# wu-kan/multicore-hw2

Hardware: AMD Instinct MI355X
Metric: queries/sec (exact 1-NN, bit-exact vs v0), m=1024 n=16777216 k=16 (higher is better)
Workload: dtype f32 results (f16 MFMA filter + f32 exact re-rank)

## Files before the change

### include/knn_mi355x.h

```cpp
#ifndef KNN_MI355X_H
#define KNN_MI355X_H

#ifdef __cplusplus
extern "C" {
#endif

void cudaCallback(int k, int m, int n, float *searchPoints, float *referencePoints,
                  int **results);

long long knn_trim(void);

typedef struct knn_index knn_index;

enum {
    KNN_OK = 0,
    KNN_EINVAL = -1,
    KNN_ENODEV = -2,
    KNN_EHIP = -3,
    KNN_ENOMEM = -4
};

#define KNN_KEY_INIT 0x7F80000000000000ull

int knn_device_count(void);
const char *knn_last_error(void);
const char *knn_version(void);

int knn_index_create(knn_index **out, int device, int k, long long n_local, const float *refs,
                     int refs_on_device, long long base_index, void *stream);
void knn_index_destroy(knn_index *idx);

typedef struct knn_geom knn_geom;
int knn_geom_create(knn_geom **out, int k, long long n_global, int nranks, const float *sample_host, long long samples,
                    int seed_tiles);
void knn_geom_destroy(knn_geom *g);
int knn_geom_info(const knn_geom *g, long long out[8]);
long long knn_geom_first_cell(const knn_geom *g, int rank);
int knn_geom_assign(const knn_geom *g, int device, const float *rows_dev, long long n, int *owner_dev, void *stream);
int knn_index_create_sharded(knn_index **out, int device, const knn_geom *g, int rank, long long n_local, const float *refs_dev,
                             const unsigned *gids_dev, void *stream);
int knn_index_seed_export(knn_index *idx, void *layer_dev, void *stream);
int knn_index_seed_attach(knn_index *idx, const void *layer_dev);

int knn_keys_init(int device, unsigned long long *keys_dev, int m, void *stream);

int knn_index_query_keys(knn_index *idx, int m, const float *queries_dev,
                         unsigned long long *keys_dev, void *stream);

int knn_index_query_keys_slot(knn_index *idx, int slot, int m, const float *queries_dev,
                              unsigned long long *keys_dev, void *stream);

#define KNN_QUERY_INIT_KEYS 1u
int knn_index_query_keys_ex(knn_index *idx, int slot, int m, const float *queries_dev,
                            unsigned long long *keys_dev, void *stream, unsigned flags);

int knn_index_query(knn_index *idx, int slot, int m, const float *queries_dev, unsigned long long *keys_dev,
                    int *indices_dev, void *stream, unsigned flags);

int knn_keys_allreduce_min(int ndev, const int *devices, unsigned long long *const *keys_dev, int m,
                           void *const *streams);

int knn_keys_to_indices(int device, const unsigned long long *keys_dev, int m, int *out_dev,
                        void *stream);

int knn_index_query_host(knn_index *idx, int m, const float *queries_host, int *out_host);

int knn_index_query_topk(knn_index *idx, int slot, int m, int K, const float *queries_dev, unsigned long long *keys_dev,
                         int *indices_dev, void *stream, unsigned flags);
int knn_keys_topk_merge(int device, int m, int K, const unsigned long long *a_dev, unsigned long long *b_dev, void *stream);
int knn_index_query_topk_host(knn_index *idx, int m, int K, const float *queries_host, int *indices_host, float *dist2_host);

int knn_set_option(const char *name, long long value);
long long knn_get_option(const char *name);

int knn_index_last_stats(knn_index *idx, long long stats[4]);

int knn_index_debug_counters(knn_index *idx, long long out[4]);

int knn_debug_shard_policy(int k, int m, long long n, int ndev);
int knn_debug_plan_shard(int k, int m, long long rows, long long out[4]);
int knn_debug_u8_row(int k, const float *row, const float *centre, float scale, double amax, unsigned char *codes, double out[2]);
int knn_debug_u8_bin_row(int k, const float *row, const float *centre, float scale, const float *w, unsigned char *codes, double *err);
int knn_debug_u8_bin_threshold(int k, const unsigned short *b_bits, float dup, float ratio, float er, float nmax, float w1, float *thr);

int knn_debug_scan_plan(int num_cu, int blocks_per_cu, unsigned nitems, int m, long long out[8]);
int knn_debug_scan_plan_ex(int num_cu, int blocks_per_cu, unsigned nitems, int m, int self_lists, long long out[8]);
int knn_debug_cells_query_plan(const long long in[14], long long out[28]);
int knn_debug_cells_topk_plan(const long long in[20], long long out[25]);
int knn_debug_seed_kth(const float *seed, int nseed, const float *wide, int nwide, int K, int pw, float *out);
int knn_debug_topk_gate(int k, float sigma, double amax, double bmax, double nmax, double u, double mq, double out[3]);
int knn_debug_filter_query_plan(const long long in[11], long long out[49]);

int knn_debug_filter_scores(knn_index *idx, int m, const float *queries_dev, float *scores_dev,
                            float *qnorm_dev, double consts[8]);

int knn_index_timing(knn_index *idx, int enable);
int knn_index_timing_read(knn_index *idx, int *launches, double *total_ms);

int knn_synth_fill_device(int device, float *dst_dev, long long count, unsigned long long seed,
                          long long first, void *stream);

#ifdef __cplusplus
}
#endif
#endif
```

### multicore_hw2_amd/__init__.py

```python
import ctypes
import os
import sys

import numpy as np

__all__ = ["lib", "lib_path", "cudaCallback", "KnnIndex", "KnnGeom", "KnnError", "KEY_INIT", "set_option",
           "get_option", "trim", "device_count", "EXPORTED_SYMBOLS", "shard_bounds", "keys_topk_merge"]

KEY_INIT = 0x7F80000000000000

EXPORTED_SYMBOLS = [
    "cudaCallback", "knn_device_count", "knn_last_error", "knn_version", "knn_index_create",
    "knn_index_destroy", "knn_keys_init", "knn_index_query_keys", "knn_keys_to_indices",
    "knn_index_query_host", "knn_set_option", "knn_get_option", "knn_index_last_stats",
    "knn_synth_fill_device", "knn_index_timing", "knn_index_timing_read",
    "knn_debug_filter_scores", "knn_index_query_keys_slot", "knn_trim", "knn_keys_allreduce_min",
    "knn_index_query_keys_ex", "knn_index_debug_counters", "knn_debug_scan_plan", "knn_debug_scan_plan_ex", "knn_debug_cells_query_plan", "knn_debug_cells_topk_plan", "knn_debug_seed_kth", "knn_debug_topk_gate", "knn_debug_filter_query_plan", "knn_debug_shard_policy", "knn_debug_plan_shard", "knn_debug_u8_row", "knn_debug_u8_bin_row", "knn_debug_u8_bin_threshold", "knn_index_query",
    "knn_geom_create", "knn_geom_destroy", "knn_geom_info", "knn_geom_assign", "knn_index_create_sharded",
    "knn_index_seed_export", "knn_index_seed_attach", "knn_geom_first_cell",
    "knn_index_query_topk", "knn_keys_topk_merge", "knn_index_query_topk_host",
]
QUERY_INIT_KEYS = 1

_HERE = os.path.dirname(os.path.abspath(__file__))
lib_path = os.environ.get("KNN_MI355X_LIB") or os.path.join(_HERE, "libknn_mi355x.so")
_lib = None


class KnnError(RuntimeError):
    pass


def lib():
    global _lib
    if _lib is not None:
        return _lib
    if not os.path.exists(lib_path):
        raise KnnError(f"{lib_path} is missing: run `python -c 'import __graft_entry__ as g; g.build()'` "
                       "(there is no CPU fallback)")
    if "torch" not in sys.modules and os.environ.get("KNN_MI355X_NO_TORCH") != "1":
        try:
            import torch
        except ImportError:
            pass
    L = ctypes.CDLL(lib_path)
    c_int, c_ll, c_vp, c_ull = ctypes.c_int, ctypes.c_longlong, ctypes.c_void_p, ctypes.c_ulonglong
    L.cudaCallback.argtypes = [c_int, c_int, c_int, c_vp, c_vp, ctypes.POINTER(ctypes.POINTER(c_int))]
    L.cudaCallback.restype = None
    L.knn_device_count.restype = c_int
    L.knn_last_error.restype = ctypes.c_char_p
    L.knn_version.restype = ctypes.c_char_p
    L.knn_index_create.argtypes = [ctypes.POINTER(c_vp), c_int, c_int, c_ll, c_vp, c_int, c_ll, c_vp]
    L.knn_index_destroy.argtypes = [c_vp]
    L.knn_index_destroy.restype = None
    L.knn_keys_init.argtypes = [c_int, c_vp, c_int, c_vp]
    L.knn_index_query_keys.argtypes = [c_vp, c_int, c_vp, c_vp, c_vp]
    L.knn_index_query_keys_slot.argtypes = [c_vp, c_int, c_int, c_vp, c_vp, c_vp]
    L.knn_index_query_keys_ex.argtypes = [c_vp, c_int, c_int, c_vp, c_vp, c_vp, ctypes.c_uint]
    L.knn_index_query.argtypes = [c_vp, c_int, c_int, c_vp, c_vp, c_vp, c_vp, ctypes.c_uint]
    L.knn_keys_to_indices.argtypes = [c_int, c_vp, c_int, c_vp, c_vp]
    L.knn_index_query_host.argtypes = [c_vp, c_int, c_vp, c_vp]
    L.knn_set_option.argtypes = [ctypes.c_char_p, c_ll]
    L.knn_get_option.argtypes = [ctypes.c_char_p]
    L.knn_get_option.restype = c_ll
    L.knn_index_last_stats.argtypes = [c_vp, ctypes.POINTER(c_ll)]
    L.knn_synth_fill_device.argtypes = [c_int, c_vp, c_ll, c_ull, c_ll, c_vp]
    L.knn_index_timing.argtypes = [c_vp, c_int]
    L.knn_debug_filter_scores.argtypes = [c_vp, c_int, c_vp, c_vp, c_vp, ctypes.POINTER(ctypes.c_double)]
    L.knn_index_timing_read.argtypes = [c_vp, ctypes.POINTER(c_int), ctypes.POINTER(ctypes.c_double)]
    L.knn_geom_create.argtypes = [ctypes.POINTER(c_vp), c_int, c_ll, c_int, c_vp, c_ll, c_int]
    L.knn_geom_destroy.argtypes = [c_vp]
    L.knn_geom_destroy.restype = None
    L.knn_geom_info.argtypes = [c_vp, ctypes.POINTER(c_ll)]
    L.knn_geom_assign.argtypes = [c_vp, c_int, c_vp, c_ll, c_vp, c_vp]
    L.knn_index_create_sharded.argtypes = [ctypes.POINTER(c_vp), c_int, c_vp, c_int, c_ll, c_vp, c_vp, c_vp]
    L.knn_index_seed_export.argtypes = [c_vp, c_vp, c_vp]
    L.knn_index_seed_attach.argtypes = [c_vp, c_vp]
    L.knn_index_query_topk.argtypes = [c_vp, c_int, c_int, c_int, c_vp, c_vp, c_vp, c_vp, ctypes.c_uint]
    L.knn_keys_topk_merge.argtypes = [c_int, c_int, c_int, c_vp, c_vp, c_vp]
    L.knn_index_query_topk_host.argtypes = [c_vp, c_int, c_int, c_vp, c_vp, c_vp]
    _lib = L
    return L


def _check(rc):
    if rc != 0:
        raise KnnError(f"knn_mi355x error {rc}: {lib().knn_last_error().decode(errors='replace')}")


def device_count():
    return lib().knn_device_count()


def set_option(name, value):
    _check(lib().knn_set_option(name.encode(), int(value)))


def get_option(name):
    return lib().knn_get_option(name.encode())

# ... 309 lines not shown
```

### multicore_hw2_amd/csrc/knn_cells.hip

```cpp
#include "knn_filter_dev.h"
#include "knn_exact_dev.h"
#include "knn_seed_kth.h"

#include <stdio.h>
#include <stdlib.h>
#include <algorithm>
#include <atomic>
#include <mutex>
#include <set>
#include <type_traits>
#include <vector>

#define CELL_MAX_BINS 16
#define CELL_TILES_PER_PASS 9

struct CellGeom {
    int k, bits, sa;
    unsigned char nb[16], shift[16];
    unsigned cell_base, ncells, nh;
};

static CellGeom cell_geom_of(const CellIndex &c, int k)
{
    CellGeom g;
// ... 784 lines not shown
        keep[w64] = 0ull;
    for (unsigned e0 = e_begin; e0 < e_end; e0 += INFLIGHT) {
        float lo[INFLIGHT];
#pragma unroll
        for (int u = 0; u < INFLIGHT; ++u) {
            const unsigned e = min(e0 + (unsigned)u, e_end - 1u);
            lo[u] = lo_tab[(size_t)s_q[e] * nl + l];
        }
#pragma unroll
        for (int u = 0; u < INFLIGHT; ++u) {
            const unsigned e = e0 + (unsigned)u;
            if (e < e_end) {
                const float lb = lo[u] + s_hv[e];
                const unsigned j = e - e_begin;
                if (!(lb > s_dq[e])) {
#pragma unroll
                    for (int w64 = 0; w64 < EPW / 64; ++w64)
                        if ((int)(j >> 6) == w64)
                            keep[w64] |= 1ull << (j & 63u);
                }
            }
        }
    }
    unsigned mine = 0u;
#pragma unroll
    for (int w64 = 0; w64 < EPW / 64; ++w64)
        mine += (unsigned)__popcll(keep[w64]);
    s_wcnt[wib][lane] = mine;
    __syncthreads();
    unsigned pos = 0u, total = 0u;
    for (int w = 0; w < CELL_MATCH_WAVES; ++w) {
        const unsigned v = s_wcnt[w][lane];
        pos += w < wib ? v : 0u;
        total += v;
    }
#pragma unroll
    for (int w64 = 0; w64 < EPW / 64; ++w64)
        for (u64 bits = keep[w64]; bits != 0ull; bits &= bits - 1ull) {
            const unsigned e = e_begin + (unsigned)w64 * 64u + (unsigned)__builtin_ctzll(bits);
            if (pos < stage)
                my_lds[pos] = s_q[e];
            else if (pos < cap)
                my_mem[pos] = s_q[e];
            ++pos;
        }
    if (wib == 0) {
        cell_counts[cell] = total;
    }
    __syncthreads();
    if (stage != 0u) {
        for (int j = wib; j < 64; j += CELL_MATCH_WAVES) {
            unsigned cj = 0u;
            for (int w = 0; w < CELL_MATCH_WAVES; ++w)
                cj += s_wcnt[w][j];
            cj = min(cj, stage);
            for (unsigned d = (unsigned)lane; d * 2u < cj; d += 64u)
                ((unsigned *)(lists + (size_t)(c0 + (unsigned)j) * cap))[d] = ((const unsigned *)(s_list + (size_t)j * lstride))[d];
        }
    }
}

#define CELL_SCAN_WAVES 12
#define CELL_SCAN_WAVES_KT2 16
#define CELL_SCAN_CHUNK 256
#define CELL_INLINE_RERANK_MAX 64u
#define CELL_PUBLISH_STEP 64u
#define CELL_BATCH_RECORD_LIMIT (1u << 19)
#define CELL_TOPK_RECORD_LIMIT (1u << 21)
#define CELL_SCAN_RUN 16

typedef _Float16 h2v __attribute__((ext_vector_type(2)));
__device__ __forceinline__ h8 cell_widen_u8(u2v w)
{
    const h2v nine = {(_Float16)9.0f, (_Float16)9.0f};
    h8 r;
#pragma unroll
    for (int i = 0; i < 4; ++i) {
        const unsigned x = __builtin_amdgcn_perm(0x48484848u, w[i >> 1], (i & 1) ? 0x04030402u : 0x04010400u);
        const h2v p = __builtin_bit_cast(h2v, x) - nine;
        r[2 * i] = p[0];
        r[2 * i + 1] = p[1];
    }
    return r;
}

template <int KT>
__device__ __forceinline__ u64 cell_tile_step(const h8 (&a)[KT], const f4v *__restrict__ my_nrm, int p, int half, const h8 (&b)[KT], float th)
{
    f16v d;
#pragma unroll
    for (int gq = 0; gq < 4; ++gq) {
        const f4v v = my_nrm[p * 8 + 2 * gq + half];
        d[4 * gq + 0] = v[0];
        d[4 * gq + 1] = v[1];
        d[4 * gq + 2] = v[2];
        d[4 * gq + 3] = v[3];
    }
#pragma unroll
    for (int kk = 0; kk < KT; ++kk)
        d = __builtin_amdgcn_mfma_f32_32x32x16_f16(a[kk], b[kk], d, 0, 0, 0);
    const float mn = min_tree16(d, th);
    return __ballot(mn < th);
}

template <int KT>
__device__ __forceinline__ u64 cell_tile_step_nif(const h8 (&a)[KT], const h8 (&b)[KT], float th)
{
    f16v d = __builtin_amdgcn_mfma_f32_32x32x16_f16(a[0], b[0], zero_acc(), 0, 0, 0);
#pragma unroll
    for (int kk = 1; kk < KT; ++kk)
        d = __builtin_amdgcn_mfma_f32_32x32x16_f16(a[kk], b[kk], d, 0, 0, 0);
    const float mn = min_tree16(d, th);
    return __ballot(mn < th);
}

#define CELL_FRAME_AMAX 16384.0f

template <bool U8 = false>
__device__ __forceinline__ void cell_centred_operand(const float *__restrict__ s_q32, int k, unsigned qid, int half, bool valid,
                                                     const float (&cc)[8], float scale, float ratio, float bmaxc, float nmaxc, float er,
                                                     float dupq, float sqdq, h8 &b, float &th)
{
#pragma clang fp contract(off)
    const f4v x0 = *(const f4v *)(s_q32 + (size_t)qid * 16 + 8 * half), x1 = *(const f4v *)(s_q32 + (size_t)qid * 16 + 8 * half + 4);
    const float x[8] = {x0[0], x0[1], x0[2], x0[3], x1[0], x1[1], x1[2], x1[3]};
    float sc[8], a = 0.0f, mq = 0.0f;
    h8 hv;
#pragma unroll
    for (int j = 0; j < 8; ++j) {
        sc[j] = (x[j] - cc[j]) * scale;
        hv[j] = (_Float16)sc[j];
        const float back = (float)hv[j];
        a = fmaxf(a, fabsf(back));
        mq = mq + back * back;
    }
    a = fmaxf(a, __shfl_xor(a, 32, KNN_WAVE));
    mq = mq + __shfl_xor(mq, 32, KNN_WAVE);
    b = hv * (_Float16)-2.0f;
    const float kf = (float)k;
    const float emax = U8 ? 4.8865e-4f * a + er * 1.000001f + 1.2220e-4f
                          : 4.8865e-4f * (a + bmaxc) + 1.2220e-4f;
    const float sqk = k <= 1 ? 1.0f : k <= 4 ? 2.0f : k <= 9 ? 3.0f : 4.0f;
    const float eta = sqk * emax, eta2 = kf * emax * emax;
    const float rho = 1.1921e-5f * (nmaxc + 16.0f * a * a) + 1.79e-7f + 4.77e-7f * nmaxc;
    const float dupc = dupq * ratio * ratio, sqdc = sqdq * ratio;
    const float P = dupc + 2.0f * eta * sqdc + eta2 + rho;
    th = (P * 1.00001f + (P + mq) * 2.4e-7f + 1e-30f) - mq * 0.999996f;
    if (!(a <= CELL_FRAME_AMAX)) {
        float a32 = 0.0f;
#pragma unroll
        for (int j = 0; j < 8; ++j)
            a32 = fmaxf(a32, fabsf(sc[j]));
        a32 = fmaxf(a32, __shfl_xor(a32, 32, KNN_WAVE));
        const float lb = a32 * 0.999f - bmaxc * 1.001f - 0.001f;
        const bool beyond = lb > 0.0f && lb * lb > dupc * 1.001f;
        b = (h8){0, 0, 0, 0, 0, 0, 0, 0};
        th = dupq > -INFINITY && !beyond ? INFINITY : -INFINITY;
    }
    if (!valid)
        th = -INFINITY;
}

#define CELL_PREP_WAVES 4
#define CELL_PREP_TILES 9
#define CELL_SEED_MAX_TILES 36u
#define CELL_SEED_MAX_TILES_CTR 144u
// ... 2083 lines not shown
        FTRY(hipEventRecord(w.ev_end, s));
    FTRY(knn_topk_filter_finish(st.k, m, K, st.ntiles * 32, base, q, r, w.records, nullptr, w.counts, w.nlists, w.slice, w.ctl_cur,
                                RerankPieces(), c.perm, st.n_outliers, st.outliers, cand, ccount, tp.ccap, keys, init_keys ? 1 : 0, s,
                                w.records + w.ovf_base, w.ctl_cur + KNN_CTL_RECORDS, w.ovf_cap, w.dup,
                                (float)(1.0 / ((double)st.sigma * (double)st.sigma)), st.ref_norms));
    return knn_exact_topk_launch(st.k, m, K, st.n, base, nullptr, q, r, keys, init_keys ? 1 : 0, part, part_bytes, num_cu, s,
                                 w.ctl_cur + KNN_CTL_FALLBACK);
}

extern "C" int knn_debug_topk_gate(int k, float sigma, double amax, double bmax, double nmax, double u, double mq, double out[3])
{
    if (k < 1 || k > 32 || !(sigma > 0.0f) || !out)
        return -1;
    const BoundConsts cst = knn_bound_consts(k, knn_kt_of(k), sigma, amax, bmax, nmax);
    double dup = 0.0;
    out[0] = knn_threshold(cst, u, mq, &dup);
    dup *= 1.0 + 1e-6;
    float dupf = (float)dup;
    if ((double)dupf < dup)
        dupf = nextafterf(dupf, INFINITY);
    out[1] = dupf;
    out[2] = knn_topk_gate(dupf, (float)(1.0 / ((double)sigma * (double)sigma)));
    return 0;
}

extern "C" int knn_debug_seed_kth(const float *seed, int nseed, const float *wide, int nwide, int K, int pw, float *out)
{
    if (nseed < 0 || nwide < 0 || (nseed && !seed) || (nwide && !wide) || K < 1 || K > KNN_TOPK_MAX || (pw != 2 && pw != 4) || !out)
        return -1;
    std::vector<float> a((size_t)(nseed + 31) / 32 * 32, INFINITY), b((size_t)(nwide + 31) / 32 * 32, INFINITY);
    std::copy(seed, seed + nseed, a.begin());
    std::copy(wide, wide + nwide, b.begin());
    *out = knn_seed_kth_host(a.data(), (int)a.size() / 32, b.data(), (int)b.size() / 32, K, pw);
    return 0;
}

extern "C" int knn_debug_u8_row(int k, const float *row, const float *centre, float scale, double amax, unsigned char *codes,
                                double out[2])
{
#pragma clang fp contract(off)
    if (k < 1 || k > 16 || !row || !centre || !codes || !out)
        return -1;
    float er = 0.0f, nmax = 0.0f;
    for (int d = 0; d < k; ++d) {
        const float v = (row[d] - centre[d]) * scale;
        float rh, e;
        codes[d] = (unsigned char)knn_u8_code(v, rh, e);
        er = std::max(er, e);
        nmax = nmax + rh * rh;
    }
    out[0] = er;
    out[1] = knn_bound_consts_u8(k, 1, scale, amax, er, nmax).eta;
    return 0;
}

extern "C" int knn_debug_u8_bin_row(int k, const float *row, const float *centre, float scale, const float *w, unsigned char *codes,
                                    double *err)
{
    if (k < 1 || k > 16 || !row || !centre || !w || !codes || !err)
        return -1;
    float er = 0.0f;
    for (int d = 0; d < k; ++d) {
        float rh, e;
        codes[d] = (unsigned char)knn_u8_bin_code(row[d], centre[d], scale, w[d], rh, e);
        er = std::max(er, e);
    }
    *err = er;
    return 0;
}

extern "C" int knn_debug_u8_bin_threshold(int k, const unsigned short *b_bits, float dup, float ratio, float er, float nmax, float w1,
                                          float *thr)
{
    if (k < 1 || k > 16 || !b_bits || !thr)
        return -1;
    h8 b0, b1;
    for (int j = 0; j < 8; ++j) {
        b0[j] = __builtin_bit_cast(_Float16, b_bits[j]);
        b1[j] = __builtin_bit_cast(_Float16, b_bits[8 + j]);
    }
    *thr = knn_u8_bin_threshold(k, b0, b1, dup, ratio, er, nmax, w1);
    return 0;
}
```

### multicore_hw2_amd/csrc/knn_cells_scan_body.inc

```
    extern __shared__ __attribute__((aligned(128))) unsigned char s_dyn[];
    constexpr int TPP = CELL_TILES_PER_PASS;
    constexpr int SW = KT == 1 && !CTR ? CELL_SCAN_WAVES : CELL_SCAN_WAVES_KT2;
    constexpr int QB = CTR ? 64 : 32 * KT;
    constexpr bool ONE_TRIP = DYN && U8 && !CTR && !SELF && KT == 1;
    h8 *s_qf = (h8 *)s_dyn;
    float *s_thr = (float *)(s_dyn + (size_t)m_padded * QB);
    f4v *s_nrm = (f4v *)(s_dyn + (size_t)m_padded * (QB + 4));
    float *s_dup = (float *)(s_dyn + (size_t)m_padded * (QB + 4) + (size_t)SW * TPP * 8 * sizeof(f4v));
    unsigned short *s_lists = (unsigned short *)(s_dup + m_padded);
    __shared__ unsigned s_flag;
    SCAN_STAMP(0);
    if (threadIdx.x == 0)
        s_flag = ctl[KNN_CTL_FALLBACK];
    const int lane = threadIdx.x & 63;
    const int wib = __builtin_amdgcn_readfirstlane((int)(threadIdx.x >> 6));
    const unsigned wave = blockIdx.x * (unsigned)SW + (unsigned)wib, nwaves = gridDim.x * (unsigned)SW;
    __shared__ unsigned s_next, s_imeta[DYN ? CELL_SCAN_CHUNK : 1], s_itb[DYN ? CELL_SCAN_CHUNK : 1], s_inq[DYN ? CELL_SCAN_CHUNK : 1];
    const unsigned per_wave = (nitems + nwaves - 1u) / nwaves;
    const unsigned i0 = 0u;
    const unsigned i1 = DYN ? (((nitems + (unsigned)CELL_SCAN_RUN - 1u) / (unsigned)CELL_SCAN_RUN + gridDim.x - 1u) / gridDim.x) *
                                  (unsigned)CELL_SCAN_RUN
                            : 0u;
    auto slot_item = [&](unsigned s) {
        const unsigned nruns = (nitems + (unsigned)CELL_SCAN_RUN - 1u) / (unsigned)CELL_SCAN_RUN;
        const unsigned rot = __umulhi(gridDim.x, 2654435769u) | 1u;
        const unsigned stripe = s / (unsigned)CELL_SCAN_RUN;
        const unsigned run = stripe * gridDim.x + (blockIdx.x + stripe * rot) % gridDim.x;
        const unsigned it = run * (unsigned)CELL_SCAN_RUN + s % (unsigned)CELL_SCAN_RUN;
        return run < nruns && it < nitems ? it : 0xFFFFFFFFu;
    };
    if constexpr (DYN) {
        const unsigned nc0 = min((unsigned)CELL_SCAN_CHUNK, i1 - i0);
        for (unsigned i = threadIdx.x; i < nc0; i += 64 * SW) {
            const unsigned it = slot_item(i0 + i);
            const u64 item = it != 0xFFFFFFFFu ? items[it] : 0ull;
            s_imeta[i] = (unsigned)(item >> 40);
            s_itb[i] = (unsigned)item;
            if constexpr (SELF)
                s_inq[i] = it != 0xFFFFFFFFu ? 1u : 0u;
            else
                s_inq[i] = it != 0xFFFFFFFFu ? cell_counts[(unsigned)(item >> 48)] : 0u;
        }
        if (threadIdx.x == 0)
            s_next = (unsigned)SW;
    }
    if constexpr (CTR) {
        const int kq = K > 0 ? K : krt;
        for (int i = threadIdx.x; i < m_padded * 16; i += 64 * SW)
            ((float *)s_dyn)[i] = (i >> 4) < m && (i & 15) < kq ? Q[(size_t)(i >> 4) * kq + (i & 15)] : 0.0f;
    } else if constexpr (U8) {
        const _Float16 rt = (_Float16)self.bin_ratio;
        for (int i = threadIdx.x; i < m_padded * 2; i += 64 * SW)
            s_qf[i] = qfg[i] * rt;
        const int kq = K > 0 ? K : krt;
        for (int i = threadIdx.x; i < m_padded; i += 64 * SW) {
            const size_t at = (size_t)(i >> 5) * 64 + (size_t)(i & 31);
            s_thr[i] = knn_u8_bin_threshold(kq, qfg[at] * rt, qfg[at + 32] * rt, self.dup[i], self.bin_ratio, self.bin_er,
                                            self.bin_nmax, self.bin_w1);
        }
    } else {
        for (int i = threadIdx.x; i < m_padded * 2 * KT; i += 64 * SW)
            s_qf[i] = qfg[i];
    }
    if constexpr (CTR || !U8)
        for (int i = threadIdx.x; i < m_padded; i += 64 * SW)
            s_thr[i] = thrg[i];
    if constexpr (SELF || CTR)
        for (int i = threadIdx.x; i < m_padded; i += 64 * SW)
            s_dup[i] = self.dup[i];
    __syncthreads();
    if (s_flag != 0u)
        return;
    SCAN_STAMP(1);
    f4v *my_nrm = s_nrm + wib * (TPP * 8);
    unsigned short *my_list = s_lists + (SELF ? wib * (int)CELL_SELF_CAP : 0);

    u64 *__restrict__ my_rec = rec + (size_t)wave * slice;
    unsigned cnt = 0u;
    bool dead = false;
    const int col = lane & 31, half = lane >> 5;
    unsigned c0 = i0, nc = min((unsigned)CELL_SCAN_CHUNK, i1 - i0), mine_dyn = (unsigned)wib;
    for (unsigned g0 = 0u;; g0 += 64u) {
        unsigned v_meta = 0u, v_tb = 0u, v_nq = 0u;
        if constexpr (DYN) {
            if (g0 == 0u && c0 >= i1)
                break;
            if (g0 != 0u && mine_dyn >= nc) {
                c0 += CELL_SCAN_CHUNK;
                if (c0 >= i1)
                    break;
                nc = min((unsigned)CELL_SCAN_CHUNK, i1 - c0);
                __syncthreads();
                for (unsigned i = threadIdx.x; i < nc; i += 64 * SW) {
                    const unsigned it = slot_item(c0 + i);
                    const u64 item = it != 0xFFFFFFFFu ? items[it] : 0ull;
                    s_imeta[i] = (unsigned)(item >> 40);
                    s_itb[i] = (unsigned)item;
                    if constexpr (SELF)
                        s_inq[i] = it != 0xFFFFFFFFu ? 1u : 0u;
                    else
                        s_inq[i] = it != 0xFFFFFFFFu ? cell_counts[(unsigned)(item >> 48)] : 0u;
                }
                if (threadIdx.x == 0)
                    s_next = (unsigned)SW;
                __syncthreads();
                mine_dyn = (unsigned)wib;
            }
            if (mine_dyn < nc && lane == 0 && !dead) {
                v_meta = s_imeta[mine_dyn];
                v_tb = s_itb[mine_dyn];
                v_nq = s_inq[mine_dyn];
            }
        } else {
            if (g0 >= per_wave || dead)
                break;
            const unsigned mine = (g0 + (unsigned)lane) * nwaves + wave;
            const bool in = g0 + (unsigned)lane < per_wave && mine < nitems;
            const u64 item = in ? items[mine] : 0ull;
            v_meta = (unsigned)(item >> 40);
            v_tb = (unsigned)item;
            if constexpr (SELF)
                v_nq = in ? 1u : 0u;
            else
                v_nq = in ? cell_counts[v_meta >> 8] : 0u;
        }
        for (u64 todo = __ballot(v_nq != 0u); todo != 0ull && !dead; todo &= todo - 1ull) {
            const int j = (int)__builtin_ctzll(todo);
            const unsigned tb = (unsigned)__builtin_amdgcn_readlane((int)v_tb, j);
            const unsigned meta = (unsigned)__builtin_amdgcn_readlane((int)v_meta, j);
            const unsigned te = tb + (meta & 0xFFu);
            const unsigned cellj = meta >> 8;
            unsigned nq;
            if constexpr (SELF) {
                __builtin_amdgcn_wave_barrier();
                nq = cell_self_list(self.lo_t, self.hi, self.sa, m_padded, cellj, m, s_dup, my_list, lane);
                wave_lds_sync();
                if (nq == 0u)
                    continue;
            } else {
                nq = (unsigned)__builtin_amdgcn_readlane((int)v_nq, j);
            }
// ... 15 lines not shown
                    unsigned hw = (unsigned)half;
                    __asm__ volatile("" : "+v"(hw));
                    wc = ((const h8 *)self.binw)[(size_t)cellj * 2 + hw];
                } else {
                    wc = ((const h8 *)self.binw)[(size_t)cellj * 2 + half];
                }
            }
            if constexpr (CTR) {
                const float *__restrict__ fr = self.frame + (size_t)cellj * KNN_CELL_FRAME_WORDS;
#pragma unroll
                for (int j = 0; j < 8; ++j)
                    ccv[j] = fr[8 * half + j];
                c_scale = fr[16];
                c_ratio = fr[17];
                c_bmax = fr[18];
                c_nmax = fr[19];
                if constexpr (U8) {
                    c_er = self.cell_u8[(size_t)cellj * 2];
                    c_nmax = self.cell_u8[(size_t)cellj * 2 + 1];
                }
            }
            for (unsigned t0 = tb; t0 < te && !dead; t0 += TPP) {
                const int nt = (int)min((unsigned)TPP, te - t0);
                h8 ar[U8 ? 1 : TPP][KT];
                u2v a8[U8 ? TPP : 1];
#pragma unroll
                for (int p = 0; p < TPP; ++p)
                    if (p < nt) {
                        if constexpr (U8) {
                            a8[p] = __builtin_nontemporal_load(&((const u2v *)rf)[(size_t)(t0 + (unsigned)p) * 64 + lane]);
                        } else {
#pragma unroll
                            for (int kk = 0; kk < KT; ++kk)
                                ar[U8 ? 0 : p][kk] = __builtin_nontemporal_load(&rf[((size_t)(t0 + (unsigned)p) * KT + kk) * 64 + lane]);
                        }
                    }
                if constexpr (!NIF) {
                    const f4v *__restrict__ rn4 = (const f4v *)rn + (size_t)t0 * 8;
                    const f4v n0 = lane < nt * 8 ? __builtin_nontemporal_load(&rn4[lane]) : (f4v){0.f, 0.f, 0.f, 0.f};
                    f4v n1 = {0.f, 0.f, 0.f, 0.f};
                    if constexpr (TPP * 8 > 64)
                        n1 = 64 + lane < nt * 8 ? __builtin_nontemporal_load(&rn4[64 + lane]) : (f4v){0.f, 0.f, 0.f, 0.f};
                    if constexpr (ONE_TRIP)
                        __asm__ volatile("" : "+v"(l0), "+v"(l1), "+v"(wc));
                    __builtin_amdgcn_wave_barrier();
                    if (TPP * 8 >= 64 || lane < TPP * 8)
                        my_nrm[lane] = n0;
                    if constexpr (TPP * 8 > 64)
                        if (lane < TPP * 8 - 64)
                            my_nrm[64 + lane] = n1;
                    wave_lds_sync();
                }
                for (unsigned q0 = 0u; q0 < nq && !dead; q0 += 32u) {
                    const unsigned idx = q0 + (unsigned)col;
                    const bool valid = idx < nq;
                    unsigned qid;
                    if constexpr (SELF) {
                        qid = dense ? (valid ? idx : 0u) : (unsigned)my_list[valid ? idx : 0u];
                    } else if (q0 < 64u) {
                        const unsigned from = __shfl(l0, (int)idx, KNN_WAVE);
                        qid = valid ? from : __shfl(l0, 0, KNN_WAVE);
                    } else if (q0 < 128u) {
                        const unsigned from = __shfl(l1, (int)(idx - 64u), KNN_WAVE);
                        qid = valid ? from : __shfl(l0, 0, KNN_WAVE);
                    } else {
                        qid = dense ? (valid ? idx : 0u) : (unsigned)list[valid ? idx : 0u];
                    }
                    if constexpr (ONE_TRIP)
                        qid = dense ? (valid ? idx : 0u) : qid;
                    h8 b[KT];
                    float th;
                    if constexpr (CTR) {
                        if (t0 == tb || nq > 32u)
                            cell_centred_operand<U8>((const float *)s_dyn, K > 0 ? K : krt, qid, half, valid, ccv, c_scale, c_ratio, c_bmax, c_nmax, c_er,
                                                 s_dup[qid], s_thr[qid], b_kept, th_kept);
                        b[0] = b_kept;
                        th = th_kept;
                    } else {
#pragma unroll
                        for (int kk = 0; kk < KT; ++kk)
                            b[kk] = s_qf[((qid >> 5) * KT + (unsigned)kk) * 64u + (unsigned)half * 32u + (qid & 31u)];
                        th = valid ? s_thr[qid] : -INFINITY;
                        if constexpr (U8) {
                            float dw = (float)b[0][0] * (float)wc[0];
#pragma unroll
                            for (int i = 1; i < 8; ++i)
                                dw = dw + (float)b[0][i] * (float)wc[i];
                            dw = dw + __shfl_xor(dw, 32, KNN_WAVE);
                            th = th - dw;
                        }
                    }
#pragma unroll
                    for (int p = 0; p < TPP; ++p) {
                        if (p < nt) {
                            u64 mask;
                            if constexpr (U8) {
                                if constexpr (!CTR)
                                    __asm__ volatile("" : "+v"(a8[p]));
                                const h8 a1[1] = {cell_widen_u8(a8[p])};
                                mask = cell_tile_step<1>(a1, my_nrm, p, half, b, th);
                            } else {
                                mask = NIF ? cell_tile_step_nif<KT>(ar[p], b, th) : cell_tile_step<KT>(ar[p], my_nrm, p, half, b, th);
                            }
                            if (__builtin_expect(mask != 0ull, 0)) {
                                const bool hit = (mask >> lane) & 1ull;
                                const unsigned pos = cnt + __builtin_amdgcn_mbcnt_hi((unsigned)(mask >> 32),
                                                                                     __builtin_amdgcn_mbcnt_lo((unsigned)mask, 0u));
                                unsigned hh = (unsigned)half;
                                if constexpr (U8 && !CTR)
                                    __asm__ volatile("" : "+v"(hh));
                                const u64 r = ((u64)qid << 32) | ((u64)(t0 + (unsigned)p) << 1) | (u64)hh;
                                if (hit && pos < slice)
                                    my_rec[pos] = r;
                                const unsigned total = cnt + (unsigned)__popcll(mask);
                                if (total > slice && ovf_cap != 0u) {
                                    const unsigned first_over = max(cnt, slice);
                                    unsigned obase = ovf_cap;
                                    if (lane == 0 && !dead)
                                        obase = atomicAdd(&ctl[KNN_CTL_RECORDS], total - first_over);
                                    obase = (unsigned)__builtin_amdgcn_readfirstlane((int)obase);
                                    if (hit && pos >= slice) {
                                        const unsigned op = obase + (pos - first_over);
                                        if (op < ovf_cap)
                                            rec[(size_t)ovf_base + op] = r;
                                    }
                                    dead = obase + (total - first_over) > ovf_cap;
                                }
                                const unsigned steps_new = (total / CELL_PUBLISH_STEP - cnt / CELL_PUBLISH_STEP) * CELL_PUBLISH_STEP;
                                cnt = total;
                                if (!SELF && steps_new != 0u && ovf_cap != 0u) {
                                    if ((wave & 63u) == 0u) {
                                        unsigned seen = 0u;
                                        if (lane == 0)
                                            seen = atomicAdd(&ctl[KNN_CTL_TOTAL], steps_new) + steps_new;
                                        seen = (unsigned)__builtin_amdgcn_readfirstlane((int)seen);
                                        if (seen > (TOPK ? CELL_TOPK_RECORD_LIMIT : CELL_BATCH_RECORD_LIMIT) / 64u) {
                                            if (lane == 0)
                                                atomicMax(&ctl[KNN_CTL_RECORDS], ovf_cap + 1u);
                                            dead = true;
                                        }
                                    } else if (__hip_atomic_load(&ctl[KNN_CTL_RECORDS], __ATOMIC_RELAXED, __HIP_MEMORY_SCOPE_AGENT) > ovf_cap) {
                                        dead = true;
                                    }
                                }
                            }
                        }
                    }
                }
            }
        }
        if constexpr (DYN) {
            unsigned nx = 0u;
            if (lane == 0)
                nx = dead ? nc : atomicAdd(&s_next, 1u);
            mine_dyn = (unsigned)__builtin_amdgcn_readfirstlane((int)nx);
        }
    }
    SCAN_STAMP(2);
    const unsigned nrec = min(cnt, slice);
    if (lane == 0)
        counts[wave] = nrec;
#ifndef KNN_CELLS_SCAN_RECORD_ONLY
    if (nrec > CELL_INLINE_RERANK_MAX && !dead && lane == 0)
        __hip_atomic_store(&ctl[KNN_CTL_DEFERRED], 1u, __ATOMIC_RELAXED, __HIP_MEMORY_SCOPE_AGENT);
    if (nrec != 0u && nrec <= CELL_INLINE_RERANK_MAX && !dead) {
        __builtin_amdgcn_fence(__ATOMIC_RELEASE, "workgroup");
        __builtin_amdgcn_fence(__ATOMIC_ACQUIRE, "workgroup");
        const int k = K > 0 ? K : krt;
        for (unsigned c0 = 0u; c0 < nrec * 16u; c0 += 64u) {
            const unsigned c = c0 + (unsigned)lane;
            const bool live = c < nrec * 16u;
            const u64 e = live ? __hip_atomic_load(&my_rec[c >> 4], __ATOMIC_RELAXED, __HIP_MEMORY_SCOPE_WORKGROUP) : 0ull;
            const unsigned qi = (unsigned)(e >> 32), lo = (unsigned)e, reg = c & 15u;
            const long long pos = (long long)(lo >> 1) * 32 + 8 * (reg >> 2) + 4 * (lo & 1u) + (reg & 3u);
            const unsigned row = live && pos < npos ? perm[pos] : 0xFFFFFFFFu;
            const float *__restrict__ qp = Q + (size_t)qi * k;
            constexpr int KD = K > 0 ? K : 16;
            const u64 cur = keys[qi];
            const float *__restrict__ rp = R + (size_t)(row != 0xFFFFFFFFu ? row : 0u) * k;
            float acc = 0.0f;
#pragma unroll
            for (int ch = 0; ch < KT; ++ch) {
// ... 48 lines not shown
```

### multicore_hw2_amd/csrc/knn_filter_dev.h

```cpp
#pragma once

#include "knn_common.h"

#include <math.h>
#include <string.h>

#ifdef KNN_NO_POOL
#define KNN_DEV_ALLOC(p, bytes) hipMalloc(p, bytes)
#define KNN_DEV_FREE(p) hipFree(p)
#else
#define KNN_DEV_ALLOC(p, bytes) knn_dev_alloc((void **)(p), bytes)
#define KNN_DEV_FREE(p) knn_dev_free((void *)(p))
#endif

#include <math.h>
#include <stdio.h>
#include <string.h>
#include <stdlib.h>
#include <algorithm>
#include <chrono>
#include <vector>

typedef _Float16 h8 __attribute__((ext_vector_type(8)));
typedef float f16v __attribute__((ext_vector_type(16)));
// ... 43 lines not shown
};

__host__ __device__ inline BoundConsts knn_bound_consts(int k, int kt, double sigma, double amax,
                                                        double bmax, double nmax)
{
    const double u = 0x1p-24;
    const double theta = 0x1p-11 + 0x1p-23;
    const double thp = theta / (1.0 - theta);
    const double nu0 = 0x1p-14 * 1.001;
    const double kp = 16.0 * kt;
    const double emax = thp * (amax + bmax) + 2.0 * nu0;
    BoundConsts c;
    c.eta2 = k * emax * emax;
    c.eta = sqrt(c.eta2);
    const double omega = kt * 0x1p-18;
    c.gam = (kp + 2.0) * u;
    const double mmax = kp * amax * amax;
    c.rho = (omega + 2.0 * c.gam) * 2.0 * (nmax + mmax) + kp * 0x1p-27;
    c.rho += 0x1p-21 * nmax + 0x1p-24;
    c.g2 = (k + 3.0) * u * 1.0001;
    c.tau = k * 0x1p-125;
    c.sigma2 = sigma * sigma;
    return c;
}

__host__ __device__ inline unsigned knn_u8_code(float v, float &rh, float &err)
{
#pragma clang fp contract(off)
    const float q = fminf(fmaxf(rintf(v * 128.0f), -128.0f), 127.0f);
    rh = q * 0.0078125f;
    err = fabsf(v - rh) + 0x1p-22f * fabsf(v) + 0x1p-100f;
    return (unsigned)((int)q + 128);
}

__host__ __device__ inline BoundConsts knn_bound_consts_u8(int k, int kt, double sigma, double amax, double er, double nmax)
{
    BoundConsts c = knn_bound_consts(k, kt, sigma, amax, 0.0, nmax);
    const double theta = 0x1p-11 + 0x1p-23;
    const double emax = theta / (1.0 - theta) * amax + er * (1.0 + 1e-6) + 2.0 * (0x1p-14 * 1.001);
    c.eta2 = k * emax * emax;
    c.eta = sqrt(c.eta2);
    return c;
}

__host__ __device__ inline unsigned knn_u8_bin_code(float x, float centre, float scale, float w, float &rh, float &err)
{
#pragma clang fp contract(off)
    const float u = (x - centre) * scale;
    const float v = u - w;
    float e;
    const unsigned b = knn_u8_code(v, rh, e);
    err = e + 0x1p-22f * fabsf(u);
    return b;
}

__host__ __device__ inline float knn_u8_bin_threshold(int k, const h8 &b0, const h8 &b1, float dup, float ratio, float er, float nmax, float w1)
{
#pragma clang fp contract(off)
    float a = 0.0f, mq = 0.0f;
#pragma unroll
    for (int j = 0; j < 16; ++j) {
        const float h = (float)(j < 8 ? b0[j & 7] : b1[j & 7]) * -0.5f;
        a = fmaxf(a, fabsf(h));
        mq = mq + h * h;
    }
    if (!(dup > -INFINITY))
        return -INFINITY;
    const float kf = (float)k;
    const float emax = 4.8865e-4f * a + er * 1.000001f + 1.2220e-4f * ratio;
    const float sqk = k <= 1 ? 1.0f : k <= 4 ? 2.0f : k <= 9 ? 3.0f : 4.0f;
    const float eta = sqk * emax, eta2 = kf * emax * emax;
    const float rho = 1.1921e-5f * (nmax + 2.0f * kf + 16.0f * a * a) + 1.79e-7f + 4.77e-7f * nmax;
    const float dupc = dup * ratio * ratio;
#ifdef __HIP_DEVICE_COMPILE__
    const float sqdc = __builtin_amdgcn_sqrtf(fmaxf(dupc, 0x1p-100f)) * 1.000001f;
#else
    const float sqdc = sqrtf(fmaxf(dupc, 0x1p-100f)) * 1.000001f;
#endif
    const float P = dupc + 2.0f * eta * sqdc + eta2 + rho;
    const float th = (P * 1.00001f + (P + mq) * 2.4e-7f + 1e-30f) - mq * 0.999996f;
    return th + (0x1p-18f * (fabsf(th) + 2.0f * a * w1) + 0x1p-14f * w1);
}

__host__ __device__ inline float knn_threshold(const BoundConsts &c, double u, double mq, double *dup_out = nullptr)
{
    double dt = u + mq * (1.0 + 1.01 * c.gam) + c.rho;
    if (dt < 0.0)
        dt = 0.0;
    const double sq0 = c.eta + sqrt(dt + 2.0 * c.eta2);
    const double dup = sq0 * sq0 * (1.0 + c.g2) * (1.0 + c.g2) + c.sigma2 * c.tau;
    if (dup_out)
        *dup_out = dup;
    double thr = dup + 2.0 * c.eta * sqrt(dup) + c.eta2 + c.rho - mq * (1.0 - c.gam);
    thr += fabs(thr) * 1e-6 + 1e-30;
    float tf = (float)thr;
    if ((double)tf < thr)
        tf = nextafterf(tf, INFINITY);
    return nextafterf(tf, INFINITY);
}


__device__ __forceinline__ float min3f(float a, float b, float c)
{
    return __builtin_fminf(__builtin_fminf(a, b), c);
}

#define FTRY(call)                       \
    do {                                 \
        hipError_t e_ = (call);          \
        if (e_ != hipSuccess)            \
            return e_;                   \
    } while (0)

static const float kAmaxLimit = 1024.0f;
```

Before: 9.276 million.

## Use raw u8 widening with threshold folding offset and MFMA weight dot

Replaces the centered u8-to-f16 widening in the non-CTR scan path with a cheaper byte-perm that yields raw code values offset by a constant, and folds the resulting bias into a new per-query threshold formula (adding 9*sum(b) and widened error margins). The per-tile weight dot product is computed with an MFMA instead of a scalar loop plus shuffle. This cuts ALU work in the hot filter loop but loosens the threshold, which may let more candidates through to exact re-rank, and it relies on the new error bounds being correct for bit-exactness.

```diff
diff --git a/include/knn_mi355x.h b/include/knn_mi355x.h
--- a/include/knn_mi355x.h
+++ b/include/knn_mi355x.h
@@ -82,6 +82,7 @@
 int knn_debug_u8_row(int k, const float *row, const float *centre, float scale, double amax, unsigned char *codes, double out[2]);
 int knn_debug_u8_bin_row(int k, const float *row, const float *centre, float scale, const float *w, unsigned char *codes, double *err);
 int knn_debug_u8_bin_threshold(int k, const unsigned short *b_bits, float dup, float ratio, float er, float nmax, float w1, float *thr);
+int knn_debug_u8_bin_threshold_raw(int k, const unsigned short *b_bits, float dup, float ratio, float er, float nmax, float w1, float *thr);
 
 int knn_debug_scan_plan(int num_cu, int blocks_per_cu, unsigned nitems, int m, long long out[8]);
 int knn_debug_scan_plan_ex(int num_cu, int blocks_per_cu, unsigned nitems, int m, int self_lists, long long out[8]);
diff --git a/multicore_hw2_amd/__init__.py b/multicore_hw2_amd/__init__.py
--- a/multicore_hw2_amd/__init__.py
+++ b/multicore_hw2_amd/__init__.py
@@ -15,7 +15,7 @@
     "knn_index_query_host", "knn_set_option", "knn_get_option", "knn_index_last_stats",
     "knn_synth_fill_device", "knn_index_timing", "knn_index_timing_read",
     "knn_debug_filter_scores", "knn_index_query_keys_slot", "knn_trim", "knn_keys_allreduce_min",
-    "knn_index_query_keys_ex", "knn_index_debug_counters", "knn_debug_scan_plan", "knn_debug_scan_plan_ex", "knn_debug_cells_query_plan", "knn_debug_cells_topk_plan", "knn_debug_seed_kth", "knn_debug_topk_gate", "knn_debug_filter_query_plan", "knn_debug_shard_policy", "knn_debug_plan_shard", "knn_debug_u8_row", "knn_debug_u8_bin_row", "knn_debug_u8_bin_threshold", "knn_index_query",
+    "knn_index_query_keys_ex", "knn_index_debug_counters", "knn_debug_scan_plan", "knn_debug_scan_plan_ex", "knn_debug_cells_query_plan", "knn_debug_cells_topk_plan", "knn_debug_seed_kth", "knn_debug_topk_gate", "knn_debug_filter_query_plan", "knn_debug_shard_policy", "knn_debug_plan_shard", "knn_debug_u8_row", "knn_debug_u8_bin_row", "knn_debug_u8_bin_threshold", "knn_debug_u8_bin_threshold_raw", "knn_index_query",
     "knn_geom_create", "knn_geom_destroy", "knn_geom_info", "knn_geom_assign", "knn_index_create_sharded",
     "knn_index_seed_export", "knn_index_seed_attach", "knn_geom_first_cell",
     "knn_index_query_topk", "knn_keys_topk_merge", "knn_index_query_topk_host",
diff --git a/multicore_hw2_amd/csrc/knn_cells.hip b/multicore_hw2_amd/csrc/knn_cells.hip
--- a/multicore_hw2_amd/csrc/knn_cells.hip
+++ b/multicore_hw2_amd/csrc/knn_cells.hip
@@ -890,6 +890,15 @@
         r[2 * i + 1] = p[1];
     }
     return r;
+}
+
+__device__ __forceinline__ h8 cell_widen_u8_raw(u2v w)
+{
+    u4v r;
+#pragma unroll
+    for (int i = 0; i < 4; ++i)
+        r[i] = __builtin_amdgcn_perm(0x48484848u, w[i >> 1], (i & 1) ? 0x04030402u : 0x04010400u);
+    return __builtin_bit_cast(h8, r);
 }
 
 template <int KT>
@@ -3139,3 +3148,17 @@
     *thr = knn_u8_bin_threshold(k, b0, b1, dup, ratio, er, nmax, w1);
     return 0;
 }
+
+extern "C" int knn_debug_u8_bin_threshold_raw(int k, const unsigned short *b_bits, float dup, float ratio, float er, float nmax, float w1,
+                                              float *thr)
+{
+    if (k < 1 || k > 16 || !b_bits || !thr)
+        return -1;
+    h8 b0, b1;
+    for (int j = 0; j < 8; ++j) {
+        b0[j] = __builtin_bit_cast(_Float16, b_bits[j]);
+        b1[j] = __builtin_bit_cast(_Float16, b_bits[8 + j]);
+    }
+    *thr = knn_u8_bin_threshold_raw(k, b0, b1, dup, ratio, er, nmax, w1);
+    return 0;
+}
diff --git a/multicore_hw2_amd/csrc/knn_cells_scan_body.inc b/multicore_hw2_amd/csrc/knn_cells_scan_body.inc
--- a/multicore_hw2_amd/csrc/knn_cells_scan_body.inc
+++ b/multicore_hw2_amd/csrc/knn_cells_scan_body.inc
@@ -55,8 +55,8 @@
         const int kq = K > 0 ? K : krt;
         for (int i = threadIdx.x; i < m_padded; i += 64 * SW) {
             const size_t at = (size_t)(i >> 5) * 64 + (size_t)(i & 31);
-            s_thr[i] = knn_u8_bin_threshold(kq, qfg[at] * rt, qfg[at + 32] * rt, self.dup[i], self.bin_ratio, self.bin_er,
-                                            self.bin_nmax, self.bin_w1);
+            s_thr[i] = knn_u8_bin_threshold_raw(kq, qfg[at] * rt, qfg[at + 32] * rt, self.dup[i], self.bin_ratio, self.bin_er,
+                                                self.bin_nmax, self.bin_w1);
         }
     } else {
         for (int i = threadIdx.x; i < m_padded * 2 * KT; i += 64 * SW)
@@ -238,12 +238,8 @@
                             b[kk] = s_qf[((qid >> 5) * KT + (unsigned)kk) * 64u + (unsigned)half * 32u + (qid & 31u)];
                         th = valid ? s_thr[qid] : -INFINITY;
                         if constexpr (U8) {
-                            float dw = (float)b[0][0] * (float)wc[0];
-#pragma unroll
-                            for (int i = 1; i < 8; ++i)
-                                dw = dw + (float)b[0][i] * (float)wc[i];
-                            dw = dw + __shfl_xor(dw, 32, KNN_WAVE);
-                            th = th - dw;
+                            const f16v pw = __builtin_amdgcn_mfma_f32_32x32x16_f16(wc, b[0], zero_acc(), 0, 0, 0);
+                            th = th - pw[0];
                         }
                     }
 #pragma unroll
@@ -253,7 +249,7 @@
                             if constexpr (U8) {
                                 if constexpr (!CTR)
                                     __asm__ volatile("" : "+v"(a8[p]));
-                                const h8 a1[1] = {cell_widen_u8(a8[p])};
+                                const h8 a1[1] = {CTR ? cell_widen_u8(a8[p]) : cell_widen_u8_raw(a8[p])};
                                 mask = cell_tile_step<1>(a1, my_nrm, p, half, b, th);
                             } else {
                                 mask = NIF ? cell_tile_step_nif<KT>(ar[p], b, th) : cell_tile_step<KT>(ar[p], my_nrm, p, half, b, th);
diff --git a/multicore_hw2_amd/csrc/knn_filter_dev.h b/multicore_hw2_amd/csrc/knn_filter_dev.h
--- a/multicore_hw2_amd/csrc/knn_filter_dev.h
+++ b/multicore_hw2_amd/csrc/knn_filter_dev.h
@@ -149,6 +149,38 @@
     return th + (0x1p-18f * (fabsf(th) + 2.0f * a * w1) + 0x1p-14f * w1);
 }
 
+__host__ __device__ inline float knn_u8_bin_threshold_raw(int k, const h8 &b0, const h8 &b1, float dup, float ratio, float er, float nmax, float w1)
+{
+#pragma clang fp contract(off)
+    float a = 0.0f, mq = 0.0f, sb = 0.0f, sa = 0.0f;
+#pragma unroll
+    for (int j = 0; j < 16; ++j) {
+        const float bj = (float)(j < 8 ? b0[j & 7] : b1[j & 7]);
+        const float h = bj * -0.5f;
+        a = fmaxf(a, fabsf(h));
+        mq = mq + h * h;
+        sb = sb + bj;
+        sa = sa + fabsf(bj);
+    }
+    if (!(dup > -INFINITY))
+        return -INFINITY;
+    const float kf = (float)k;
+    const float emax = 4.8865e-4f * a + er * 1.000001f + 1.2220e-4f * ratio;
+    const float sqk = k <= 1 ? 1.0f : k <= 4 ? 2.0f : k <= 9 ? 3.0f : 4.0f;
+    const float eta = sqk * emax, eta2 = kf * emax * emax;
+    const float rho = 1.1921e-5f * (nmax + 32.0f * kf * a) + 1.79e-7f + 4.77e-7f * nmax;
+    const float dupc = dup * ratio * ratio;
+#ifdef __HIP_DEVICE_COMPILE__
+    const float sqdc = __builtin_amdgcn_sqrtf(fmaxf(dupc, 0x1p-100f)) * 1.000001f;
+#else
+    const float sqdc = sqrtf(fmaxf(dupc, 0x1p-100f)) * 1.000001f;
+#endif
+    const float P = dupc + 2.0f * eta * sqdc + eta2 + rho;
+    const float th = (P * 1.00001f + (P + mq) * 2.4e-7f + 1e-30f) - mq * 0.999996f;
+    const float t9 = th + 9.0f * sb;
+    return t9 + (1.1921e-5f * (2.0f * a * w1) + 0x1.2p-16f * sa + 0x1p-21f * (fabsf(t9) + 2.0f * a * w1));
+}
+
 __host__ __device__ inline float knn_threshold(const BoundConsts &c, double u, double mq, double *dup_out = nullptr)
 {
     double dt = u + mq * (1.0 + 1.01 * c.gam) + c.rho;
```

Result: faster. 9.552 million, median of 6 (+3.0%).
